# tenstack/batch-scheduler

Hardware: AMD Instinct MI355X
Metric: pod x node fit evals/sec (higher is better)
Workload: dtype int64; 1 GPU; cfg3/tail: 10000 pods / 2000 groups / 5000 nodes, 5 int64 lanes (cpu, mem, eph, pods, gpu), seed 20260921; stages=prefilter+filter+tally+ready, parallelism=single GPU

## Files before the change

### batch-scheduler_amd/build.py

```python
from __future__ import annotations

import os
import shutil
import subprocess

HERE = os.path.dirname(os.path.abspath(__file__))
CSRC = os.path.join(HERE, "csrc")
LIB_DIR = os.environ.get("BS_LIB_DIR") or HERE
PREBUILT_ONLY = bool(os.environ.get("BS_LIB_DIR"))
LIB_PATH = os.path.join(LIB_DIR, "libbsched.so")
_COMMON = ["bs_common.hpp", "bs_kernels.hpp", "bs_nodew_layout.hpp", "bs_lanes.hpp", os.path.join("..", "..", "include", "bsched.h")]
_CTX = _COMMON + ["bs_ctx.hpp", "bs_carve.hpp", "bs_hostmem.hpp", "bs_pod_ranges.hpp"]
_FAST = ["bs_launch.hpp", "bs_fast.hpp", "bs_filter_t.hpp"]
_SEQ = _CTX + ["bs_seq.hpp"]
UNITS = {
    "bsched.hip": _CTX + _FAST + ["bs_epoch.hpp", "bs_queue.hpp", "bs_fdeny.hpp", "bs_sort.hpp", "bs_fit.hpp"],
    "tu_fast.hip": _COMMON + _FAST,
    "tu_seq.hip": _SEQ,
    "tu_seq_expire.hip": _SEQ + ["bs_seq_expire.hpp", "bs_seq_expire_list.hpp"],
    "tu_preempt.hip": _CTX + ["bs_preempt.hpp", "bs_preempt_commit.hpp", "bs_preempt_commit_gang.hpp", "bs_preempt_gang_runs.hpp", "bs_preempt_geom.hpp", "bs_bound_apply.hpp",
                              "bs_bound_nodes.hpp", "bs_bound_nodes_replay.hpp", "bs_pdb.hpp"],
}
SOURCES = list(UNITS)
LATER_UNITS = {
    "tu_wait.hip": _SEQ + ["bs_wait.hpp", "bs_wait_list.hpp", "bs_bound_nodes_replay.hpp"],
}
ALL_UNITS = {**UNITS, **LATER_UNITS}
ALL_SOURCES = list(ALL_UNITS)
LIST_UNITS = {
    "tu_groups.hip": _CTX + ["bs_groups_list.hpp", "bs_groups_list_check.hpp"],
}
BUILD_UNITS = {**ALL_UNITS, **LIST_UNITS}
BUILD_SOURCES = list(BUILD_UNITS)
HEADERS = sorted({h for hs in BUILD_UNITS.values() for h in hs})
OBJ_DIR = os.path.join(HERE, "build")
FLAGS = ["--offload-arch=gfx950", "-O3", "-std=c++17", "-fPIC", "-ffp-contract=off",
         "-fno-fast-math", "-Wall", "-Wno-unused-function"]


def hipcc() -> str:
    exe = shutil.which("hipcc") or "/opt/rocm/bin/hipcc"
    if not os.path.exists(exe):
        raise RuntimeError("hipcc not found: the gfx950 library cannot be built")
    return exe
# ... 103 lines not shown
```

### batch-scheduler_amd/csrc/bs_ctx.hpp

```cpp
#pragma once
#include <rccl/rccl.h>

#include <algorithm>
#include <string>
#include <vector>

#include "bs_carve.hpp"
#include "bs_hostmem.hpp"
#include "bs_kernels.hpp"
#include "bs_lanes.hpp"
#include "bs_pod_ranges.hpp"

namespace bs {

struct EventPair { hipEvent_t a, b; uint32_t id; };

inline size_t align256(size_t x) { return (x + 255) & ~(size_t)255; }
template <class T>
T* at(T* p, size_t n) { return p ? p + n : nullptr; }

struct PodLayout {
  Piece<int32_t> group;
  Piece<int64_t> req;
  Piece<uint32_t> pres, cls, pclass, ppair;
// ... 95 lines not shown
  Piece<uint32_t> off_gmm, off_gsc, off_gmatched, off_gcls, off_gmrpres;
  Piece<uint8_t> off_gflags;
  Piece<int64_t> off_gminres;
  Piece<uint64_t> off_gocc;
  size_t gpack_bytes = 0;
  int32_t info_tag = 0, kinfo_tag = 0;
  bool info_pending = false, kinfo_pending = false;
  uint32_t max_group_cls = 0, max_pod_cls = 0;
  uint32_t h_K = 0;
  uint32_t k_bound = 0;

  uint32_t P = 0;
  DevBuf d_pack[2], d_outpack;
  PodLayout lay[2], stage_lay;
  uint32_t cur_pack = 0;
  bool last_use_classes = false;
  uint32_t map_p = 0;
  DevBuf d_gstat2, d_cdir, d_pdir, d_ckeys, d_cpres, d_pkeys;
  uint32_t gstat_cur = 0;
  uint32_t pair_cap = 0, dir_slots = 0;
  uint32_t ids_used = 0;
  bool rep_valid = false;
  bool dirs_ready = false;
  uint32_t id_room = 0;
  uint32_t serial_insert_max = 2048;
  uint64_t n_applies = 0, n_rederives = 0;
  Piece<uint8_t> off_pf_code, off_fl_code, off_ready;
  Piece<uint32_t> off_pf_first_k, off_fl_feasible, off_fl_slot, off_admit;
  Piece<int32_t> off_pf_leader;
  size_t outpack_bytes = 0;

  DevBuf d_first_elig, d_first_owner, d_first_reject, d_first_pod, d_cap_epoch;
  DevBuf d_epoch, d_nepochs, d_leader_epoch, d_panic_epoch;
  DevBuf d_tcode, d_stage, d_leader_raw, d_first_row, d_first_row64, d_scan_rec, d_feas_rec, d_chunk_rec, d_qreq_s, d_qflags_s, d_qpos;
  DevBuf d_needed, d_qcount, d_ticket, d_desc;
  bool scratch_armed = false;
  bool side_ready = false;
  DevBuf d_tables, d_kp, d_stats, d_fparams, d_fflags, d_chunk_tot, d_blk_scratch, d_gmax, d_chunk_kp;
  DevBuf d_cls_slots, d_cls_rep, d_cls_id, d_qtab_s, d_fu_slot, d_uparams, d_uflags, d_uclaim, d_fu_bitmap, d_fu_feas;
  DevBuf d_nodew;
  bool batch_void = false;
  uint32_t tp_tmin = 768;
  bool no_nodew = false;
  uint32_t slot_keep = 0xFFFFFFFFu;
  uint32_t cls_cap = 0, hash_keep = 0x7FFFFFFFu, n_nominres = 0, scan_slots_cap = 0, filter_slots_cap = 0;
  DevBuf d_fl_bitmap, d_admit, d_ready, d_gcount, d_admit64, d_own_start;
  bool owner_ready = false;
  DevBuf d_order_rank, d_sort;
  uint32_t order_g = 0;
  DevBuf d_gstat, d_pair_next, d_pair_firstq, d_first_reach, d_qstamp_s, d_fast_reject, d_epoch_group;
  bool pairs_ready = false;
  bool bitmap_valid = false;
  bool last_fast = false;
  bool batch_since_pods = false;
  size_t off_hfeas = 0, off_htag = 0;
  uint32_t hstride = 0;
  int32_t host_tag = 0;
  bool last_host_out = false;
  uint32_t no_fast = 0;
  DevBuf d_run_of_epoch, d_run_leader, d_gslot, d_gfirstq;
  bool epochs_ready = false, einfo_pending = false;
  int32_t einfo_tag = 0;
  uint32_t h_R = 0, h_eflags = 0, no_epoch = 0;
  uint32_t last_chain = 0;
  uint32_t last_rows = 0;
  DevBuf d_sq;
// ... 122 lines not shown
```

### batch-scheduler_amd/csrc/bs_fast.hpp

```cpp
#pragma once

#include "bs_kernels.hpp"
#include "bs_filter_t.hpp"

#ifdef BS_NT_TABLES
#define BS_TBL_STORE(p, v) __builtin_nontemporal_store((v), (p))
#else
#define BS_TBL_STORE(p, v) (*(p) = (v))
#endif
namespace bs {

template <bool INL = false>
__device__ __forceinline__ void arm_tally(const GroupsDev& gr, const BatchDev& b, const BatchParams& prm, uint32_t i, uint32_t nthreads);

__device__ __forceinline__ const uint8_t* range_glocal(const BatchDev& b) { return reinterpret_cast<const uint8_t*>(b.pod_ranges); }
__device__ __forceinline__ const uint32_t* range_start(const BatchDev& b, uint32_t G) { return b.pod_ranges + (G + 3u) / 4u; }
__device__ __forceinline__ const uint32_t* range_lfirst(const BatchDev& b, uint32_t G, uint32_t pod_blocks) { return range_start(b, G) + pod_blocks + 1u; }
__device__ __forceinline__ bool range_local_on(const BatchDev& b, const BatchParams& prm) {
  return b.pod_ranges && prm.do_tally && prm.do_ready && !prm.filter_deny;
}

#if BS_EMIT_MAIN
__global__ void k_pods_prep(unsigned long long* tables, uint32_t ntab, uint32_t* gstat, uint32_t ngstat, uint32_t* kcount, uint32_t* gcount, uint32_t G) {
  const uint32_t t = blockIdx.x * blockDim.x + threadIdx.x, nt = gridDim.x * blockDim.x;
// ... 31 lines not shown
  bool winner;
  const uint32_t r = dedupe_insert(slots, mask, hash_keep, h, i, [&](uint32_t o) { return o < pods.p && pods.group[o] == gi && id[rep[o]] == c; }, winner);
  ppair[i] = r;
  if (winner) {
    unsigned long long* head = reinterpret_cast<unsigned long long*>(gstat + (((size_t)3 * G + 1) & ~(size_t)1)) + gi;
    pair_next[i] = atomicExch(head, ((unsigned long long)c << 32) | i);
  }
}
#endif

#if BS_EMIT_MAIN
__global__ void k_groups_apply(const GroupDelta* d, uint32_t n, uint32_t* matched, uint32_t* status_scheduled, uint8_t* flags) {
  const uint32_t t = blockIdx.x * blockDim.x + threadIdx.x;
  if (t >= n) return;
  const GroupDelta x = d[t];
  matched[x.index] = x.matched;
  status_scheduled[x.index] = x.status_scheduled;
  flags[x.index] = (uint8_t)x.flags;
}
#endif

__device__ __forceinline__ void leader_publish(const GroupsDev& gr, const BatchDev& b, uint32_t C, int32_t tag, int32_t* info, int32_t l, int32_t pn,
                                               uint32_t l_matched, uint8_t l_flags, uint32_t l_cls) {
  int32_t steady = -1;
  if (!pn && l >= 0 && C && l_matched > 0 && (l_flags & BS_GROUP_HAS_POD) && l_cls < C) {
    steady = (int32_t)(C + l_cls);
    TableDesc d;
    d.cls = l_cls;
    d.pct = 0.7f;
    b.desc[steady] = d;
  }
  b.leader_epoch[0] = l;
  b.panic_epoch[0] = pn ? 1 : 0;
  __hip_atomic_store(&info[0], l, __ATOMIC_RELAXED, __HIP_MEMORY_SCOPE_SYSTEM);
  __hip_atomic_store(&info[1], pn, __ATOMIC_RELAXED, __HIP_MEMORY_SCOPE_SYSTEM);
  __hip_atomic_store(&info[2], steady, __ATOMIC_RELAXED, __HIP_MEMORY_SCOPE_SYSTEM);
  asm volatile("s_waitcnt vmcnt(0)" ::: "memory");
  __hip_atomic_store(&info[3], tag, __ATOMIC_RELAXED, __HIP_MEMORY_SCOPE_SYSTEM);
}

__device__ __forceinline__ void leader_info_block(const GroupsDev& gr, const BatchDev& b, uint32_t C, int32_t tag, int32_t* info, const DeltaPack& dp,
                                                  uint32_t* matched, uint32_t* status_scheduled, uint8_t* flags) {
  __shared__ unsigned long long s_w[kLeaderBlock / 64];
  __shared__ uint32_t s_slow;
  if (threadIdx.x < dp.n) {
    const GroupDelta x = dp.d[threadIdx.x];
    matched[x.index] = x.matched;
    status_scheduled[x.index] = x.status_scheduled;
    flags[x.index] = (uint8_t)x.flags;
  }
  if (threadIdx.x == 0) s_slow = 0;
  __syncthreads();
  if (!gr.g) {
    if (threadIdx.x == 0) leader_publish(gr, b, C, tag, info, -1, 0, 0u, 0, 0u);
    return;
  }
  if (gr.g <= (uint32_t)kLeaderBlock * kLeaderPerThread) {
    uint32_t f_[kLeaderPerThread], mm_[kLeaderPerThread], sc_[kLeaderPerThread], ma_[kLeaderPerThread], cl_[kLeaderPerThread];
#pragma unroll
    for (int it = 0; it < kLeaderPerThread; ++it) {
      const uint32_t g = threadIdx.x + (uint32_t)it * kLeaderBlock;
      f_[it] = mm_[it] = sc_[it] = ma_[it] = cl_[it] = 0;
      if (g < gr.g) { f_[it] = gr.flags[g]; mm_[it] = gr.min_member[g]; sc_[it] = gr.status_scheduled[g]; ma_[it] = gr.matched[g]; cl_[it] = gr.cls[g]; }
    }
    unsigned long long best = 0;
    bool panic = false;
// ... 125 lines not shown

struct LeaderPre { Res mr; bool have_mr; int64_t min_member, status_scheduled, matched; };
template <bool PUB, typename T>
__device__ __forceinline__ void st_pub(T* p, T v) {
  if constexpr (PUB) __hip_atomic_store(p, v, __ATOMIC_RELAXED, __HIP_MEMORY_SCOPE_AGENT);
  else *p = v;
}
#ifndef BS_HOME_WT
#define BS_HOME_WT 0
#endif
template <typename T>
__device__ __forceinline__ void st_home(T* p, T v) {
#if BS_HOME_WT
  __hip_atomic_store(p, v, __ATOMIC_RELAXED, __HIP_MEMORY_SCOPE_SYSTEM);
#else
  *p = v;
#endif
}
__device__ __forceinline__ uint32_t ld_agent(const uint32_t* p) { return __hip_atomic_load(p, __ATOMIC_RELAXED, __HIP_MEMORY_SCOPE_AGENT); }
__device__ __forceinline__ unsigned long long ld_agent64(const void* p) {
  return __hip_atomic_load(reinterpret_cast<const unsigned long long*>(p), __ATOMIC_RELAXED, __HIP_MEMORY_SCOPE_AGENT);
}
template <int TS>
__device__ __forceinline__ void leader_pre_load(const GroupsDev& gr, int32_t leader, Shape<TS> sh, LeaderPre& o) {
  const uint32_t l = leader >= 0 ? (uint32_t)leader : 0u;
#pragma unroll
  for (uint32_t j = 0; j < BS_MAX_LANES; ++j) o.mr.v[j] = j < sh.L() ? gr.minres[(size_t)j * gr.g + l] : 0;
  o.mr.present = gr.mrpres[l];
  o.have_mr = (gr.flags[l] & BS_GROUP_HAS_MINRES) != 0;
  o.min_member = (int64_t)gr.min_member[l];
  o.status_scheduled = (int64_t)gr.status_scheduled[l];
  o.matched = (int64_t)gr.matched[l];
}
template <int TS>
__device__ __forceinline__ void pre_allocated_from(const LeaderPre& lp, Shape<TS> sh, uint32_t gate, Res& out) {
  res_zero(out, sh);
  const int64_t mm = lp.min_member;
  const int64_t not_finished = lp.matched != 0 ? mm - lp.matched : mm - lp.status_scheduled;
  if (not_finished > 0 && lp.have_mr) {
    Res times;
#pragma unroll
    for (uint32_t j = 0; j < BS_MAX_LANES; ++j)
      if (j < sh.L()) times.v[j] = wmul(lp.mr.v[j], not_finished);
    times.present = lp.mr.present;
    res_add(out, times, sh, gate);
  }
  if (out.v[BS_LANE_PODS] == 0) out.v[BS_LANE_PODS] = mm + 1;
}
template <int TS>
__device__ __forceinline__ uint32_t filter_slot_values(const Res& cur_in, const LeaderPre& lp, Shape<TS> sh, uint32_t gate, int64_t (&R)[4], int64_t (&M)[4]) {
  Res ms, cur = cur_in;
  res_zero(ms, sh);
  res_add(ms, lp.mr, sh, gate);
  res_add(cur, ms, sh, gate);
  uint32_t ff = 0;
#pragma unroll
  for (uint32_t s = 0; s < BS_MAX_SCALARS; ++s) {
    if (s < sh.S()) {
      if ((cur.present & (1u << s)) && cur.v[4 + s] != 0) ff |= 1u;
      if ((ms.present & (1u << s)) && ms.v[4 + s] != 0) ff |= 2u;
    }
  }
#pragma unroll
  for (int j = 0; j < 4; ++j) { R[j] = cur.v[j]; M[j] = ms.v[j]; }
  return ff;
}
// ... 269 lines not shown
                                                 const int64_t* ckeys, const uint32_t* cpres, uint32_t kcap, bool direct = false, uint32_t forced_cls = 0) {
  __shared__ unsigned long long s_wtot[BS_MAX_LANES][4];
  __shared__ uint32_t s_kp[BS_MAX_SCALARS];
  __shared__ unsigned long long s_off[BS_MAX_LANES];
  __shared__ uint32_t s_kpg[BS_MAX_SCALARS];
  __shared__ int64_t s_req[kStepSlotsMax][BS_MAX_LANES];
  __shared__ uint32_t s_qf[kStepSlotsMax];
  __shared__ uint32_t s_first[kStepSlotsMax];
  BS_STAMP(2, 0);
  const Shape<TS> sh(prm.S);
  const uint32_t L = sh.L(), S = sh.S(), LP = prm.LP;
  const uint32_t k = chunk * kTblChunk + threadIdx.x;
  const bool in_range = REGS ? k < nd.n : k < nd.m;
  const uint32_t n = REGS ? (in_range ? k : 0u) : (in_range ? nd.kmap[k] : 0u);
  const TableDesc d = REGS ? TableDesc{forced_cls, 0.7f} : *forced;
  const uint32_t fw = nd.fit[(size_t)d.cls * nd.fit_words + (n >> 5)];
  const uint8_t fl = nd.flags[n];
  const bool valid = in_range && (!REGS || !(fl & BS_NODE_SKIP_MASK));
  const uint32_t ap = nd.apres[n], rp = nd.rpres[n];
  int64_t al[BS_MAX_LANES], rq[BS_MAX_LANES];
#pragma unroll
  for (uint32_t j = 0; j < BS_MAX_LANES; ++j) {
    if (j < L) {
      al[j] = nd.alloc[(size_t)j * nd.stride + n];
      rq[j] = nd.req[(size_t)j * nd.stride + n];
    }
  }
  const uint32_t K = prm.k_host ? prm.k_host : *b.kclass;
  const uint32_t per = (K + nshares - 1u) / nshares, s_lo = share * per, s_hi = min(K, s_lo + per);
  Res raw;
  int32_t leader0 = -1;
  uint8_t panic0 = 0;
  LeaderPre lp0{};
  if constexpr (REGS) {
    const uint32_t cc = s_lo + threadIdx.x < s_hi ? s_lo + threadIdx.x : 0u;
#pragma unroll
    for (uint32_t j = 0; j < BS_MAX_LANES; ++j)
      if (j < L) raw.v[j] = ckeys[(size_t)j * kcap + cc];
    raw.present = cpres[cc];
    leader0 = b.leader_epoch[0];
    panic0 = b.panic_epoch[0];
    if (gr.g) leader_pre_load(gr, leader0, sh, lp0);
  }
  const bool fit = valid && ((fw >> (n & 31u)) & 1u) && !(fl & BS_NODE_TAINT_ERR);
  const uint32_t pres = fit ? (ap & rp) : 0u;
  if (threadIdx.x < BS_MAX_SCALARS) s_kp[threadIdx.x] = BS_INF;
  for (uint32_t t = threadIdx.x; t < kStepSlotsMax; t += kTblChunk) s_first[t] = BS_INF;
  unsigned long long incl[BS_MAX_LANES];
  const int w = wave_id();
#pragma unroll
  for (uint32_t j = 0; j < BS_MAX_LANES; ++j) {
    incl[j] = 0;
    if (j < L) {
      const bool live = fit && (j < 4 || (pres & (1u << (j - 4)))) && !(j == BS_LANE_EPH && !prm.eph_gate);
      const unsigned long long left = live ? (unsigned long long)wsub(scale_f32(al[j], d.pct), rq[j]) : 0ull;
      incl[j] = wave_incl_scan_add_u64(left);
      if (lane_id() == 63) s_wtot[j][w] = incl[j];
    }
  }
  __syncthreads();
#pragma unroll
  for (uint32_t s2 = 0; s2 < BS_MAX_SCALARS; ++s2) {
    if (s2 < S) {
      const unsigned long long mk = __ballot(valid && (pres & (1u << s2)));
      if (mk && lane_id() == 0) atomicMin(&s_kp[s2], chunk * kTblChunk + (uint32_t)(threadIdx.x & ~63u) + (uint32_t)(__ffsll((long long)mk) - 1));
    }
  }
#pragma unroll
  for (uint32_t j = 0; j < BS_MAX_LANES; ++j) {
    if (j < L) {
      unsigned long long off = 0, tot = 0;
#pragma unroll
      for (int i = 0; i < 4; ++i) {
        const unsigned long long x = s_wtot[j][i];
        if (i < w) off += x;
        tot += x;
      }
      incl[j] += off;
      if (threadIdx.x == 0 && share == 0) {
        if constexpr (REGS) {
          const unsigned long long tag = (unsigned long long)prm.seq_inv << 32;
          st_pub<true>(&b.chunk_rec[(size_t)chunk * kRecStride + 2u * j], tag | (uint32_t)tot);
          st_pub<true>(&b.chunk_rec[(size_t)chunk * kRecStride + 2u * j + 1u], tag | (uint32_t)(tot >> 32));
        } else {
          st_pub<true>(&b.chunk_tot[(size_t)chunk * 16 + j], tot);
        }
      }
    }
  }
  __syncthreads();
  __shared__ uint32_t s_ok;
  if constexpr (REGS) {
    if (share == 0 && threadIdx.x < S) st_pub<true>(&b.chunk_rec[(size_t)chunk * kRecStride + 16u + threadIdx.x], ((unsigned long long)prm.seq_inv << 32) | s_kp[threadIdx.x]);
    BS_STAMP(2, 1);
  } else {
    if (share == 0 && threadIdx.x < 16) st_pub<true>(&b.chunk_kp[(size_t)chunk * 16 + threadIdx.x], threadIdx.x < BS_MAX_SCALARS ? s_kp[threadIdx.x] : BS_INF);
    asm volatile("s_waitcnt vmcnt(0)" ::: "memory");
    __syncthreads();
    BS_STAMP(2, 1);
    if (threadIdx.x == 0 && share == 0) (void)__hip_atomic_fetch_add(&b.ticket[kTkTab], 1u, __ATOMIC_RELAXED, __HIP_MEMORY_SCOPE_AGENT);
  }
  if constexpr (REGS) {
    const uint32_t t = s_lo + threadIdx.x;
    if (t < s_hi) {
      uint32_t qf = 0x80000000u;
      Res q;
      res_zero(q, sh);
      if (leader0 >= 0 && !panic0) {
        Res cur;
        res_zero(cur, sh);
        res_add(cur, raw, sh, prm.eph_gate);
        qf = class_scan_query(cur, lp0, sh, prm.eph_gate, q);
      }
      s_qf[threadIdx.x] = qf;
#pragma unroll
      for (uint32_t j = 0; j < BS_MAX_LANES; ++j)
        if (j < L) s_req[threadIdx.x][j] = q.v[j];
    }
  }
  if constexpr (!REGS) {
    if (threadIdx.x == 0) s_ok = (step_wait(&b.ticket[kTkTab], tk_tab0, nchunks, b.h_err) && step_wait(&b.ticket[kTkSlots], tk_pods0, pod_blocks, b.h_err)) ? 1u : 0u;
    __syncthreads();
    BS_STAMP(2, 2);
    if (!s_ok) return;
  }
  {
    const uint32_t ch = (uint32_t)lane_id();
    unsigned long long cv[BS_MAX_LANES];
    uint32_t ckp[BS_MAX_SCALARS];
    if constexpr (REGS) {
      if (w == 0) {
        const uint32_t tagw = prm.seq_inv;
        const unsigned long long* rec = b.chunk_rec + (size_t)(ch < nchunks ? ch : 0u) * kRecStride;
        bool ok = false;
        for (uint32_t spins = 0;; ++spins) {
// ... 128 lines not shown
    BS_STAMP(2, 7);
    return;
  }
  for (uint32_t t = threadIdx.x; t < nmine; t += kTblChunk) {
    if (s_first[t] == BS_INF) continue;
    atomicMin(&b.first_row[s_lo + t], s_first[t]);
  }
  BS_STAMP(2, 7);
}

__device__ __forceinline__ void step_filter_split(uint32_t K, uint32_t W, uint32_t target_waves, uint32_t& tiles, uint32_t& bpw, uint32_t& nchunk) {
  tiles = (2u * K + 63u) / 64u;
  uint32_t nsplit = max(1u, target_waves / max(tiles, 1u));
  nsplit = min(nsplit, max((W + 1u) / 2u, 1u));
  bpw = max(2u, (((W + nsplit - 1u) / nsplit + 1u) / 2u) * 2u);
  nchunk = (W + bpw - 1u) / bpw;
  if ((nchunk + 3u) / 4u > kFeasRecGroups) {
    bpw = ((W + 4u * kFeasRecGroups - 1u) / (4u * kFeasRecGroups) + 1u) / 2u * 2u;
    nchunk = (W + bpw - 1u) / bpw;
  }
}
template <int TS>
__device__ __forceinline__ void step_filter_block(const GroupsDev& gr, const NodesDev& nd, const BatchDev& b, const BatchParams& prm, const int64_t* ckeys,
                                                  const uint32_t* cpres, uint32_t kcap, uint32_t target_waves, uint32_t ustride, uint32_t bx, uint32_t nblocks,
                                                  bool direct, uint32_t tk_slots0, uint32_t slot_producers) {
  __shared__ uint32_t s_cnt[4][64];
  BS_STAMP_AT(4, 0, bx);
  const Shape<TS> sh(prm.S);
  const uint32_t gate = prm.eph_gate, K = prm.k_host ? prm.k_host : (uint32_t)__builtin_amdgcn_readfirstlane((int)*b.kclass), U = 2u * K;
  const uint32_t W = (nd.n + 63u) / 64u;
  if (!U || !W) return;
  uint32_t tiles, bpw, nchunk;
  step_filter_split(K, W, target_waves, tiles, bpw, nchunk);
  const uint32_t groups = (nchunk + 3u) / 4u;
  const int32_t leader0 = b.leader_epoch[0];
  LeaderPre lp0{}, lp1{};
  const bool two = prm.sop_leader0 >= 0 && prm.sop_leader0 != leader0;
  if (gr.g) {
    leader_pre_load(gr, leader0, sh, lp0);
    if (two) leader_pre_load(gr, prm.sop_leader0, sh, lp1); else lp1 = lp0;
  }
  bool waited = false;
  for (uint32_t bi = bx; bi < tiles * groups; bi += nblocks) {
    const uint32_t tile = bi % tiles, group = bi / tiles, chunk = group * 4u + (uint32_t)wave_id();
    const uint32_t src = tile * 64u + (uint32_t)lane_id();
    const bool second = src >= K;
    const uint32_t c = src < U ? (second ? src - K : src) : 0u;
    uint32_t cnt = 0;
    if (chunk < nchunk) {
      Res raw;
#pragma unroll
      for (uint32_t j = 0; j < BS_MAX_LANES; ++j)
        if (j < sh.L()) raw.v[j] = ckeys[(size_t)j * kcap + c];
      raw.present = cpres[c];
      Res cur;
      res_zero(cur, sh);
      res_add(cur, raw, sh, gate);
      LeaderPre lp = lp0;
      if (second) lp = lp1;
      const bool on = src < U && (second ? prm.sop_leader0 >= 0 : leader0 >= 0) && lp.have_mr;
      int64_t R[4], M[4];
      const uint32_t ff = filter_slot_values(cur, lp, sh, gate, R, M);
      filter_item<2, 4, true, true>(nd, b, U, ustride, tile, chunk * bpw, min(W, chunk * bpw + bpw), 0u,
                                    on ? (ff | ((uint32_t)BS_FL_EVALUATED << 8)) : ((uint32_t)BS_FL_NOT_RUN << 8), R, M, &cnt);
    }
    s_cnt[wave_id()][lane_id()] = cnt;
    BS_STAMP_AT(4, 1, bx);
    if (direct && b.h_rows) asm volatile("s_waitcnt vmcnt(0)" ::: "memory");
    __syncthreads();
    BS_STAMP_AT(4, 2, bx);
    if (wave_id() == 0 && src < U) {
      const uint32_t sum = s_cnt[0][lane_id()] + s_cnt[1][lane_id()] + s_cnt[2][lane_id()] + s_cnt[3][lane_id()];
      if (direct) {
        st_pub<true>(&b.feas_rec[(size_t)group * (2u * kStepSlotsMax) + src], ((unsigned long long)prm.seq_inv << 32) | sum);
      } else {
        if (!waited) { (void)step_wait(&b.ticket[kTkSlots], tk_slots0, slot_producers, b.h_err); waited = true; }
        if (sum) atomicAdd(&b.fu_feas[src], sum);
      }
    }
    __syncthreads();
  }
  BS_STAMP_AT(4, 7, bx);
}

template <int TS>
__device__ __forceinline__ void class_slots_block(const GroupsDev& gr, const BatchDev& b, const BatchParams& prm, const int64_t* ckeys, const uint32_t* cpres,
                                                  uint32_t kcap, uint32_t blk, bool zero_feas) {
  const Shape<TS> sh(prm.S);
#ifdef BS_TEST_OLD_ZERO
  zero_feas = true;
#endif
  const uint32_t gate = prm.eph_gate, K = prm.k_host ? prm.k_host : *b.kclass;
  const uint32_t c = blk * kTblChunk + threadIdx.x;
  Res raw;
  const uint32_t cc = c < K ? c : 0u;
#pragma unroll
  for (uint32_t j = 0; j < BS_MAX_LANES; ++j)
    if (j < sh.L()) raw.v[j] = ckeys[(size_t)j * kcap + cc];
  raw.present = cpres[cc];
  const int32_t leader0 = b.leader_epoch[0];
  const uint8_t panic0 = b.panic_epoch[0];
  LeaderPre lp0{}, lp1{};
  const bool two = prm.run_filter && prm.sop_leader0 >= 0 && prm.sop_leader0 != leader0;
  if (gr.g) {
    leader_pre_load(gr, leader0, sh, lp0);
    if (two) leader_pre_load(gr, prm.sop_leader0, sh, lp1); else lp1 = lp0;
  }
  if (c < K) {
    Res cur;
    res_zero(cur, sh);
    res_add(cur, raw, sh, gate);
    if (leader0 >= 0 && !panic0) {
      Res q;
      const uint32_t qfw = class_scan_query(cur, lp0, sh, gate, q);
      int64_t* dst = b.qreq_s + (size_t)c * prm.LP;
#pragma unroll
      for (uint32_t j = 0; j < BS_MAX_LANES; ++j)
        if (j < prm.LP) st_pub<true>(&dst[j], j < sh.L() ? q.v[j] : (int64_t)INT64_MIN);
      st_pub<true>(&b.qflags_s[c], qfw);
      st_pub<true>(&b.qtab_s[c], (int32_t)0);
      st_pub<true>(&b.first_row[c], BS_INF);
      st_pub<true>(&b.qstamp_s[c], prm.stamp);
    }
    if (prm.run_filter) {
      if (leader0 >= 0) filter_slot_from<TS, true>(b, prm, cur, lp0, sh, gate, c, zero_feas);
      if (prm.sop_leader0 >= 0) filter_slot_from<TS, true>(b, prm, cur, lp1, sh, gate, c + K, zero_feas);
    }
  }
  BS_STAMP(1, 4);
  asm volatile("s_waitcnt vmcnt(0)" ::: "memory");
  __syncthreads();
  BS_STAMP(1, 5);
  if (threadIdx.x == 0) (void)__hip_atomic_fetch_add(&b.ticket[kTkSlots], 1u, __ATOMIC_RELAXED, __HIP_MEMORY_SCOPE_AGENT);
}


template <bool INL>
__device__ __forceinline__ void arm_tally(const GroupsDev& gr, const BatchDev& b, const BatchParams& prm, uint32_t i, uint32_t nthreads) {
  if (i == 0) __hip_atomic_store(&b.ticket[1], 0u, __ATOMIC_RELAXED, __HIP_MEMORY_SCOPE_AGENT);
// ... 572 lines not shown
```

### batch-scheduler_amd/csrc/bs_kernels.hpp

```cpp
#pragma once

#include "bs_common.hpp"
#include "bs_nodew_layout.hpp"

namespace bs {

struct NodesDev {
  uint32_t n, stride;
  const int64_t* alloc;
  const int64_t* req;
  const uint32_t* apres;
  const uint32_t* rpres;
  const uint8_t* flags;
  const uint32_t* fit;
  uint32_t fit_words, n_classes;
  const uint32_t* kmap;
  uint32_t m;
  const int64_t* left4;
  const int64_t* lglob;
};

struct GroupsDev {
  uint32_t g;
  const uint32_t* min_member;
  const uint32_t* status_scheduled;
  const uint32_t* matched;
  const uint8_t* flags;
  const uint32_t* cls;
  const int64_t* minres;
  const uint32_t* mrpres;
  const uint64_t* occupied;
};

struct PodsDev {
  uint32_t p;
// ... 13 lines not shown
inline uint32_t cdiv(uint32_t a, uint32_t b) { return (a + b - 1) / b; }

struct BoundLayout { size_t boff, prio, start, group, id, req, pres, pdb, nviol; };
__host__ __device__ inline size_t bound_layout(uint32_t L, uint32_t N, uint32_t B, BoundLayout& b) {
  const size_t nB = B ? B : 1u, nN = N ? N : 1u, m = ~(size_t)255;
  size_t o = 0;
  b.boff = o; o = (o + ((size_t)N + 1) * 4 + 255) & m;
  b.prio = o; o = (o + nB * 4 + 255) & m;
  b.start = o; o = (o + nB * 8 + 255) & m;
  b.group = o; o = (o + nB * 4 + 255) & m;
  b.id = o; o = (o + nB * 4 + 255) & m;
  b.req = o; o = (o + nB * L * 8 + 255) & m;
  b.pres = o; o = (o + nB * 4 + 255) & m;
  b.pdb = o; o = (o + nB + 255) & m;
  b.nviol = o; o = (o + nN * 4 + 255) & m;
  return o;
}

constexpr uint8_t ST_ELIG = 1;
constexpr uint8_t ST_REACH6 = 2;
constexpr uint8_t ST_OWNED = 4;
constexpr uint8_t ST_QUERY = 8;

struct BatchDev {
  uint32_t* first_elig;
  uint32_t* first_owner;
  uint32_t* first_reject;
  uint32_t* first_pod;
  uint32_t* cap_epoch;
  uint32_t* epoch;
  uint32_t* nepochs;
  int32_t* leader_epoch;
  uint8_t* panic_epoch;
  uint8_t* tcode;
  uint8_t* stage;
  int32_t* leader_raw;
  uint32_t* first_row;
  unsigned long long* chunk_rec;
  unsigned long long* first_row64;
  unsigned long long* scan_rec;
  unsigned long long* feas_rec;
  int64_t* qreq_s;
  uint32_t* qflags_s;
  uint32_t* qpos;
  uint32_t* needed;
  uint32_t* qcount;
  uint32_t* ticket;
  TableDesc* desc;
  uint32_t* ntables;
  int64_t* tables;
  uint32_t* kp;
  uint64_t* stats;
  unsigned long long* chunk_tot;
  uint32_t* chunk_kp;
  uint32_t* blk_scratch;
  int64_t* gmax;
  int64_t* fparams;
  uint32_t* fflags;
  const uint32_t* pclass;
  const uint32_t* kclass;
  unsigned long long* cls_slots;
  uint32_t cls_mask;
  int32_t* qtab_s;
  uint32_t* fu_slot;
  int64_t* uparams;
  uint32_t* uflags;
// ... 1467 lines not shown
BS_DEF_FILTER_POD2(1, 1, 0, 0, 0)
BS_DEF_FILTER_POD2(2, 0, 1, 0, 0)
BS_DEF_FILTER_POD2(3, 1, 1, 0, 0)
BS_DEF_FILTER_POD2(4, 0, 0, 1, 0)
BS_DEF_FILTER_POD2(5, 1, 0, 1, 0)
BS_DEF_FILTER_POD2(6, 0, 1, 1, 0)
BS_DEF_FILTER_POD2(7, 1, 1, 1, 0)
BS_DEF_FILTER_POD2(8, 0, 0, 0, 1)
BS_DEF_FILTER_POD2(9, 1, 0, 0, 1)
BS_DEF_FILTER_POD2(10, 0, 1, 0, 1)
BS_DEF_FILTER_POD2(11, 1, 1, 0, 1)
BS_DEF_FILTER_POD2(12, 0, 0, 1, 1)
BS_DEF_FILTER_POD2(13, 1, 0, 1, 1)
BS_DEF_FILTER_POD2(14, 0, 1, 1, 1)
BS_DEF_FILTER_POD2(15, 1, 1, 1, 1)

template <int MASK, int PU = 4>
__device__ __forceinline__ void filter_pod_loop(uint32_t np, const int64_t (*sR)[4], const unsigned long long (&okmask)[2],
                                                const int64_t (&l)[2][4], uint32_t (&vlo)[2], uint32_t (&vhi)[2]) {
  for (uint32_t pp = 0; pp < np; pp += PU) {
    int64_t R[PU][4];
#pragma unroll
    for (int u = 0; u < PU; ++u) {
      const uint32_t pu = min(pp + (uint32_t)u, np - 1);
#pragma unroll
      for (int j = 0; j < 4; ++j) R[u][j] = ((MASK >> j) & 1) ? sR[pu][j] : 0;
    }
#pragma unroll
    for (int u = 0; u < PU; ++u)
      filter_pod2<MASK>(min(pp + (uint32_t)u, np - 1), R[u], okmask[0], okmask[1], l[0], l[1], vlo[0], vhi[0], vlo[1], vhi[1]);
  }
}

template <int NB, int PU = 4, bool DB = true, bool REGS = false>
__device__ __forceinline__ void filter_item(const NodesDev& nd, const BatchDev& b, uint32_t U, uint32_t ustride, uint32_t ptile,
                                            uint32_t w0, uint32_t w1, uint32_t stamp = 0, uint32_t ff_in = 0, const int64_t* R_in = nullptr,
                                            const int64_t* M_in = nullptr, uint32_t* cnt_out = nullptr) {
  static_assert(NB == 2, "the inner statement handles two node blocks");
  typedef const __attribute__((address_space(4))) uint32_t* cflag_t;
  const int lane = lane_id();
  const uint32_t p0 = ptile * 64u;
  const uint32_t np = min(64u, U - p0);

  const bool mine = (uint32_t)lane < np;
  const uint32_t src = p0 + (uint32_t)lane;
  uint32_t myff = (uint32_t)BS_FL_NOT_RUN << 8;
  int64_t M[4] = {0, 0, 0, 0}, myR[4] = {0, 0, 0, 0};
  if constexpr (REGS) {
    if (mine) {
      myff = ff_in;
#pragma unroll
      for (int j = 0; j < 4; ++j) { myR[j] = R_in[j]; M[j] = M_in[j]; }
    }
  } else if (mine) {
    myff = b.uflags[src];
    const int64_t* rs = b.uparams + (size_t)src * 8;
#pragma unroll
    for (int j = 0; j < 4; ++j) { myR[j] = rs[j]; M[j] = rs[4 + j]; }
  }
  int64_t gl[8];
#pragma unroll
  for (int j = 0; j < 8; ++j) gl[j] = nd.lglob[j];
  int64_t l[NB][4], ln[NB][4];
  uint8_t nfl[NB], nfln[NB];
  auto load_blocks = [&](uint32_t w, int64_t (&dst)[NB][4], uint8_t (&fl)[NB]) {
#pragma unroll
    for (int nb = 0; nb < NB; ++nb) {
      const uint32_t n = (w + nb) * 64u + (uint32_t)lane;
      const bool nvalid = (w + nb) < w1 && n < nd.n;
      fl[nb] = 0xFF;
#pragma unroll
      for (int j = 0; j < 4; ++j) dst[nb][j] = INT64_MIN;
      if (nvalid) {
#pragma unroll
        for (int j = 0; j < 4; ++j) dst[nb][j] = nd.left4[(size_t)j * nd.stride + n];
        fl[nb] = nd.flags[n];
      }
    }
  };
  load_blocks(w0, l, nfl);
  if (!REGS && stamp) myff = (myff >> 16) == stamp ? (myff & 0xFFFFu) : ((uint32_t)BS_FL_NOT_RUN << 8);
  const uint32_t myfl = myff >> 8;
  const bool ev = myfl == BS_FL_EVALUATED;
  if (!ev) {
#pragma unroll
    for (int j = 0; j < 4; ++j) M[j] = 0;
  }
  __shared__ int64_t s_R[4][64][4];
  __builtin_amdgcn_wave_barrier();
  uint32_t lane_mask = 0;
  bool tile_allfail = false;
  {
#pragma unroll
    for (int j = 0; j < 4; ++j) s_R[wave_id()][lane][j] = myR[j];
    __builtin_amdgcn_wave_barrier();
    const bool c2pod = ev && !(myff & 1u);
    const unsigned long long c2mask = __ballot(c2pod);
#pragma unroll
    for (int j = 0; j < 4; ++j) {
      if (__ballot(c2pod && !(gl[j] >= myR[j]))) lane_mask |= 1u << j;
      if (c2mask && !__ballot(c2pod && gl[4 + j] >= myR[j])) tile_allfail = true;
    }
  }
  const unsigned long long evmask = __ballot(ev);
  if (!evmask) return;
  bool uniformM = true;
  int64_t M0[4] = {0, 0, 0, 0};
  uint32_t lb0 = 0;
  if (evmask) {
    const int first = __ffsll((long long)evmask) - 1;
    bool same = true;
#pragma unroll
    for (int j = 0; j < 4; ++j) {
// ... 331 lines not shown
```

### batch-scheduler_amd/csrc/bsched.hip

```cpp
#include <dlfcn.h>
#include <hip/hip_runtime.h>

#include <algorithm>
#include <cstdio>
#include <cstdlib>
#include <cstring>
#include <new>
#include <string>
#include <vector>

#ifndef BS_UNITY
#define BS_TU_MAIN
#endif
#include "bs_ctx.hpp"
#include "bs_fast.hpp"
#include "bs_epoch.hpp"
#include "bs_sort.hpp"
#include "bs_fit.hpp"
#include "bs_queue.hpp"
#include "bs_fdeny.hpp"
#include "bs_launch.hpp"
#ifdef BS_UNITY
#include "tu_fast.hip"
#include "tu_seq.hip"
// ... 57 lines not shown
    if (_rc) return _rc;                                       \
    __VA_ARGS__;                                               \
    LAUNCHCHK(ctx, id);                                        \
    _rc = timer_end(ctx, _slot, st);                           \
    if (_rc) return _rc;                                       \
  } while (0)
#define TIMED(ctx, id, ...) TIMED_ON(ctx, id, (hipStream_t) nullptr, __VA_ARGS__)

void advance_batch_seq(bs_ctx* c) {
  c->batch_seq++;
  c->stamp_ctr = (c->stamp_ctr + 1u) % 65535u;
  if (c->key_seq >= 0xFFFFFFFEu) { c->key_seq = 1; c->rekey_pending = true; }
  else c->key_seq++;
}

int flush_groups(bs_ctx* c);
template <class D>
void pod_cols(D& p, const PodLayout& l, void* pk) {
  p.group = l.group.in(pk); p.req = l.req.in(pk); p.pres = l.pres.in(pk); p.cls = l.cls.in(pk); p.owner = l.owner.in(pk); p.flags = l.flags.in(pk);
}
uint32_t* ppair_dev(const bs_ctx* c) { return c->lay[c->cur_pack].ppair.in(c->d_pack[c->cur_pack].p); }
uint32_t* gstat_dev(const bs_ctx* c) { return (c->gstat_cur ? c->d_gstat2 : c->d_gstat).as<uint32_t>(); }
BatchDev batch_dev(const bs_ctx* c) {
  BatchDev b{};
  b.first_elig = c->d_first_elig.as<uint32_t>();
  b.first_owner = c->d_first_owner.as<uint32_t>();
  b.first_reject = c->d_first_reject.as<uint32_t>();
  b.first_pod = c->d_first_pod.as<uint32_t>();
  b.cap_epoch = c->d_cap_epoch.as<uint32_t>();
  b.epoch = c->d_epoch.as<uint32_t>();
  b.nepochs = c->d_nepochs.as<uint32_t>();
  b.leader_epoch = c->d_leader_epoch.as<int32_t>();
  b.panic_epoch = c->d_panic_epoch.as<uint8_t>();
  b.tcode = c->d_tcode.as<uint8_t>();
  b.stage = c->d_stage.as<uint8_t>();
  b.leader_raw = c->d_leader_raw.as<int32_t>();
  b.first_row = c->d_first_row.as<uint32_t>();
  b.first_row64 = c->d_first_row64.as<unsigned long long>();
  b.scan_rec = c->d_scan_rec.as<unsigned long long>();
  b.feas_rec = c->d_feas_rec.as<unsigned long long>();
  b.chunk_rec = c->d_chunk_rec.as<unsigned long long>();
  b.qreq_s = c->d_qreq_s.as<int64_t>();
  b.qflags_s = c->d_qflags_s.as<uint32_t>();
  b.qpos = c->d_qpos.as<uint32_t>();
  b.needed = c->d_needed.as<uint32_t>();
  b.qcount = c->d_qcount.as<uint32_t>();
  b.ticket = c->d_ticket.as<uint32_t>();
  b.gcount = c->d_gcount.as<uint32_t>();
  b.own_start = c->d_own_start.as<uint32_t>();
  b.admit64 = c->d_admit64.as<unsigned long long>();
  b.desc = c->d_desc.as<TableDesc>();
  b.tables = c->d_tables.as<int64_t>();
  b.kp = c->d_kp.as<uint32_t>();
  b.stats = c->d_stats.as<uint64_t>();
  b.chunk_tot = c->d_chunk_tot.as<unsigned long long>();
  b.blk_scratch = c->d_blk_scratch.as<uint32_t>();
  b.gmax = c->d_gmax.as<int64_t>();
  b.chunk_kp = c->d_chunk_kp.as<uint32_t>();
  b.fparams = c->d_fparams.as<int64_t>();
  b.fflags = c->d_fflags.as<uint32_t>();
  b.pclass = pclass_dev(c);
  b.kclass = at(c->d_nepochs.as<uint32_t>(), 2);
  b.cls_slots = c->d_cls_slots.as<unsigned long long>();
  b.cls_mask = c->cls_cap ? c->cls_cap - 1 : 0;
  b.qtab_s = c->d_qtab_s.as<int32_t>();
  b.uparams = c->d_uparams.as<int64_t>();
// ... 640 lines not shown
int bs_create(const bs_config* cfg, bs_ctx** out) {
  if (!cfg || !out) return BS_ERR_INVALID;
  *out = nullptr;
  if (cfg->abi_version != BS_ABI_VERSION || cfg->scalar_lanes > BS_MAX_SCALARS) return BS_ERR_INVALID;
  int ndev = 0;
  if (hipGetDeviceCount(&ndev) != hipSuccess || ndev <= 0 || cfg->device < 0 || cfg->device >= ndev) return BS_ERR_NO_DEVICE;
  hipDeviceProp_t prop;
  if (hipGetDeviceProperties(&prop, cfg->device) != hipSuccess) return BS_ERR_NO_DEVICE;
  if (std::strncmp(prop.gcnArchName, "gfx950", 6) != 0) return BS_ERR_NO_DEVICE;
  bs_ctx* c = new (std::nothrow) bs_ctx();
  if (!c) return BS_ERR_NOMEM;
  c->cfg = *cfg;
  c->S = cfg->scalar_lanes;
  c->L = BS_FIXED_LANES + c->S;
  c->LP = c->S == 0 ? 4 : (c->S <= 4 ? 8 : 16);
  if (hipSetDevice(cfg->device) != hipSuccess || hipStreamCreateWithFlags(&c->stream.h, hipStreamNonBlocking) != hipSuccess ||
      hipStreamCreateWithFlags(&c->stream3.h, hipStreamNonBlocking) != hipSuccess ||
      hipEventCreateWithFlags(&c->ev_query.h, hipEventDisableTiming) != hipSuccess ||
      hipEventCreateWithFlags(&c->ev_filter.h, hipEventDisableTiming) != hipSuccess) {
    delete c;
    return BS_ERR_NO_DEVICE;
  }
  if (c->d_nepochs.reserve(64) != hipSuccess || hipMemset(c->d_nepochs.p, 0, 64) != hipSuccess || c->d_ticket.reserve(kTkWords * 4) != hipSuccess ||
      hipMemset(c->d_ticket.p, 0, kTkWords * 4) != hipSuccess) {
    delete c;
    return BS_ERR_NOMEM;
  }
  if (c->d_info.reserve(64) != hipSuccess || c->d_first_reach.reserve(64) != hipSuccess || hipMemset(c->d_first_reach.p, 0xFF, 64) != hipSuccess ||
      c->h_info.reserve(64) != hipSuccess) {
    delete c;
    return BS_ERR_NOMEM;
  }
  std::memset(c->h_info.p, 0, 64);
  c->batch_seq = 1;
  read_env_switches(c);
  *out = c;
  return BS_OK;
}

int bs_destroy(bs_ctx* c) {
  if (!c) return BS_OK;
  if (c->host_probe && c->hp_n)
    std::fprintf(stderr, "[bs host probe] %llu fast-chain batches: to chain choice %.2f us | to launch A %.2f | launch A call %.2f | to launch B %.2f | launch B call %.2f | rest %.2f\n",
                 (unsigned long long)c->hp_n, c->hp_ns[0] / 1e3 / c->hp_n, c->hp_ns[1] / 1e3 / c->hp_n, c->hp_ns[2] / 1e3 / c->hp_n, c->hp_ns[3] / 1e3 / c->hp_n,
                 c->hp_ns[4] / 1e3 / c->hp_n, c->hp_ns[5] / 1e3 / c->hp_n);
  (void)hipSetDevice(c->cfg.device);
  (void)hipStreamSynchronize(c->stream);
  (void)hipStreamSynchronize(c->stream3);
  for (auto& e : c->events) { (void)hipEventDestroy(e.a); (void)hipEventDestroy(e.b); }
  if (c->comm && c->rccl_destroy) (void)c->rccl_destroy((ncclComm_t)c->comm);
  delete c;
  return BS_OK;
}

int bs_nodes_load(bs_ctx* c, const bs_nodes_soa* nodes) {
  if (c) c->seq_wait_valid = false;
  if (!c || !nodes) return BS_ERR_INVALID;
  int rc = use_device(c);
  if (rc) return rc;
  if ((rc = settle_pending(c))) return rc;
  c->steady_prev = -1;
  const uint32_t N = nodes->n, L = c->L;
  if (N && (!nodes->allocatable || !nodes->requested || !nodes->allocatable_present || !nodes->requested_present || !nodes->flags))
    return BS_ERR_INVALID;
  if (N > 0x7FFFFFF0u) return BS_ERR_CAPACITY;
  c->N = N;
// ... 2131 lines not shown
```

Baseline: 3736 billion evals/s.

## Publish leader record as one cache line and prefetch next filter item

The kernel that picks the epoch leader now also writes a 128-byte LeaderRec holding the leader's minres, flags and counters. Downstream filter and tally kernels read that record with one coalesced per-lane load plus readlane, instead of doing several scattered group-table loads after the leader is known. The step filter loop also loads the next item's pod keys and node blocks into registers before processing the current one, and it peeks at the slot ticket so it can skip the wait when the producers are already done. The cost is more register pressure and extra code paths, with a fallback to the full load whenever the record does not match the leader or the lane count is too large.

```diff
diff --git a/batch-scheduler_amd/build.py b/batch-scheduler_amd/build.py
--- a/batch-scheduler_amd/build.py
+++ b/batch-scheduler_amd/build.py
@@ -9,7 +9,7 @@
 LIB_DIR = os.environ.get("BS_LIB_DIR") or HERE
 PREBUILT_ONLY = bool(os.environ.get("BS_LIB_DIR"))
 LIB_PATH = os.path.join(LIB_DIR, "libbsched.so")
-_COMMON = ["bs_common.hpp", "bs_kernels.hpp", "bs_nodew_layout.hpp", "bs_lanes.hpp", os.path.join("..", "..", "include", "bsched.h")]
+_COMMON = ["bs_common.hpp", "bs_kernels.hpp", "bs_nodew_layout.hpp", "bs_leader_rec.hpp", "bs_lanes.hpp", os.path.join("..", "..", "include", "bsched.h")]
 _CTX = _COMMON + ["bs_ctx.hpp", "bs_carve.hpp", "bs_hostmem.hpp", "bs_pod_ranges.hpp"]
 _FAST = ["bs_launch.hpp", "bs_fast.hpp", "bs_filter_t.hpp"]
 _SEQ = _CTX + ["bs_seq.hpp"]
diff --git a/batch-scheduler_amd/csrc/bs_ctx.hpp b/batch-scheduler_amd/csrc/bs_ctx.hpp
--- a/batch-scheduler_amd/csrc/bs_ctx.hpp
+++ b/batch-scheduler_amd/csrc/bs_ctx.hpp
@@ -151,6 +151,7 @@
 
   DevBuf d_first_elig, d_first_owner, d_first_reject, d_first_pod, d_cap_epoch;
   DevBuf d_epoch, d_nepochs, d_leader_epoch, d_panic_epoch;
+  DevBuf d_leader_rec;
   DevBuf d_tcode, d_stage, d_leader_raw, d_first_row, d_first_row64, d_scan_rec, d_feas_rec, d_chunk_rec, d_qreq_s, d_qflags_s, d_qpos;
   DevBuf d_needed, d_qcount, d_ticket, d_desc;
   bool scratch_armed = false;
diff --git a/batch-scheduler_amd/csrc/bs_fast.hpp b/batch-scheduler_amd/csrc/bs_fast.hpp
--- a/batch-scheduler_amd/csrc/bs_fast.hpp
+++ b/batch-scheduler_amd/csrc/bs_fast.hpp
@@ -87,6 +87,21 @@
   }
   b.leader_epoch[0] = l;
   b.panic_epoch[0] = pn ? 1 : 0;
+  if (b.leader_rec) {
+    LeaderRec r{};
+    r.leader = l;
+    r.panic = pn ? 1u : 0u;
+    if (l >= 0) {
+#pragma unroll
+      for (uint32_t j = 0; j < kLeaderRecLanes; ++j) r.minres[j] = j < b.leader_rec_lanes ? gr.minres[(size_t)j * gr.g + (uint32_t)l] : 0;
+      r.mrpres = gr.mrpres[l];
+      r.flags = gr.flags[l];
+      r.min_member = gr.min_member[l];
+      r.status_scheduled = gr.status_scheduled[l];
+      r.matched = gr.matched[l];
+    }
+    *b.leader_rec = r;
+  }
   __hip_atomic_store(&info[0], l, __ATOMIC_RELAXED, __HIP_MEMORY_SCOPE_SYSTEM);
   __hip_atomic_store(&info[1], pn, __ATOMIC_RELAXED, __HIP_MEMORY_SCOPE_SYSTEM);
   __hip_atomic_store(&info[2], steady, __ATOMIC_RELAXED, __HIP_MEMORY_SCOPE_SYSTEM);
@@ -278,6 +293,41 @@
   o.status_scheduled = (int64_t)gr.status_scheduled[l];
   o.matched = (int64_t)gr.matched[l];
 }
+__device__ __forceinline__ uint32_t leader_rec_fetch(const BatchDev& b) { return reinterpret_cast<const uint32_t*>(b.leader_rec)[lane_id() & 31]; }
+__device__ __forceinline__ uint32_t lane_word(uint32_t w, int lane) { return (uint32_t)__builtin_amdgcn_readlane((int)w, lane); }
+template <int TS>
+__device__ __forceinline__ void leader_pre_from_words(uint32_t w, Shape<TS> sh, LeaderPre& o) {
+#pragma unroll
+  for (uint32_t j = 0; j < BS_MAX_LANES; ++j) {
+    o.mr.v[j] = 0;
+    if (j < kLeaderRecLanes && j < sh.L())
+      o.mr.v[j] = (int64_t)(((unsigned long long)lane_word(w, kLrMinres + 2 * (int)j + 1) << 32) | lane_word(w, kLrMinres + 2 * (int)j));
+  }
+  o.mr.present = lane_word(w, kLrMrpres);
+  o.have_mr = (lane_word(w, kLrFlags) & BS_GROUP_HAS_MINRES) != 0;
+  o.min_member = (int64_t)lane_word(w, kLrMinMember);
+  o.status_scheduled = (int64_t)lane_word(w, kLrScheduled);
+  o.matched = (int64_t)lane_word(w, kLrMatched);
+}
+template <int TS>
+__device__ __forceinline__ bool leader_pre_from_rec(uint32_t w, int32_t leader0, Shape<TS> sh, LeaderPre& o) {
+  if (sh.L() > kLeaderRecLanes || (int32_t)lane_word(w, kLrLeader) != leader0) return false;
+  leader_pre_from_words(w, sh, o);
+  return true;
+}
+__device__ __forceinline__ uint32_t leader_live_fetch(const GroupsDev& gr, int32_t leader, uint32_t L, uint32_t& flags) {
+  const uint32_t l = leader >= 0 ? (uint32_t)leader : 0u;
+  const int i = lane_id() & 31;
+  const uint32_t j = min((uint32_t)(i >= kLrMinres ? (i - kLrMinres) >> 1 : 0), min(L, kLeaderRecLanes) - 1u);
+  const uint32_t* p = reinterpret_cast<const uint32_t*>(gr.minres + (size_t)j * gr.g + l) + (i >= kLrMinres ? (i - kLrMinres) & 1 : 0);
+  if (i == kLrMrpres) p = gr.mrpres + l;
+  if (i == kLrMinMember) p = gr.min_member + l;
+  if (i == kLrScheduled) p = gr.status_scheduled + l;
+  if (i == kLrMatched) p = gr.matched + l;
+  flags = gr.flags[l];
+  return *p;
+}
+__device__ __forceinline__ uint32_t leader_live_words(uint32_t w, uint32_t flags) { return lane_id() == kLrFlags ? flags : w; }
 template <int TS>
 __device__ __forceinline__ void pre_allocated_from(const LeaderPre& lp, Shape<TS> sh, uint32_t gate, Res& out) {
   res_zero(out, sh);
@@ -613,6 +663,7 @@
   int32_t leader0 = -1;
   uint8_t panic0 = 0;
   LeaderPre lp0{};
+  uint32_t lrec = 0;
   if constexpr (REGS) {
     const uint32_t cc = s_lo + threadIdx.x < s_hi ? s_lo + threadIdx.x : 0u;
 #pragma unroll
@@ -621,7 +672,7 @@
     raw.present = cpres[cc];
     leader0 = b.leader_epoch[0];
     panic0 = b.panic_epoch[0];
-    if (gr.g) leader_pre_load(gr, leader0, sh, lp0);
+    lrec = leader_rec_fetch(b);
   }
   const bool fit = valid && ((fw >> (n & 31u)) & 1u) && !(fl & BS_NODE_TAINT_ERR);
   const uint32_t pres = fit ? (ap & rp) : 0u;
@@ -682,6 +733,7 @@
     if (threadIdx.x == 0 && share == 0) (void)__hip_atomic_fetch_add(&b.ticket[kTkTab], 1u, __ATOMIC_RELAXED, __HIP_MEMORY_SCOPE_AGENT);
   }
   if constexpr (REGS) {
+    if (!leader_pre_from_rec(lrec, leader0, sh, lp0) && gr.g) leader_pre_load(gr, leader0, sh, lp0);
     const uint32_t t = s_lo + threadIdx.x;
     if (t < s_hi) {
       uint32_t qf = 0x80000000u;
@@ -876,27 +928,44 @@
   if (!U || !W) return;
   uint32_t tiles, bpw, nchunk;
   step_filter_split(K, W, target_waves, tiles, bpw, nchunk);
-  const uint32_t groups = (nchunk + 3u) / 4u;
+  const uint32_t groups = (nchunk + 3u) / 4u, items = tiles * groups;
+  auto item_fetch = [&](uint32_t bi, Res& raw, FilterPre<2>& pre) {
+    const uint32_t tile = bi % tiles, chunk = min((bi / tiles) * 4u + (uint32_t)wave_id(), nchunk - 1u);
+    const uint32_t src = tile * 64u + (uint32_t)lane_id();
+    const uint32_t c = src < U ? (src >= K ? src - K : src) : 0u;
+#pragma unroll
+    for (uint32_t j = 0; j < BS_MAX_LANES; ++j)
+      if (j < sh.L()) raw.v[j] = ckeys[(size_t)j * kcap + c];
+    raw.present = cpres[c];
+    filter_item_preload<2>(nd, chunk * bpw, min(W, chunk * bpw + bpw), pre);
+  };
+  if (bx >= items) return;
   const int32_t leader0 = b.leader_epoch[0];
+  const uint32_t lrec = leader_rec_fetch(b);
+  const bool carried = prm.sop_leader0 >= 0 && gr.g;
+  uint32_t lfl = 0;
+  const uint32_t llive = carried ? leader_live_fetch(gr, prm.sop_leader0, sh.L(), lfl) : 0u;
+  Res raw0;
+  FilterPre<2> pre0;
+  item_fetch(bx, raw0, pre0);
   LeaderPre lp0{}, lp1{};
-  const bool two = prm.sop_leader0 >= 0 && prm.sop_leader0 != leader0;
-  if (gr.g) {
-    leader_pre_load(gr, leader0, sh, lp0);
-    if (two) leader_pre_load(gr, prm.sop_leader0, sh, lp1); else lp1 = lp0;
+  const bool two = carried && prm.sop_leader0 != leader0;
+  if (!leader_pre_from_rec(lrec, leader0, sh, lp0) && gr.g) leader_pre_load(gr, leader0, sh, lp0);
+  if (two) {
+    if (sh.L() <= kLeaderRecLanes) leader_pre_from_words(leader_live_words(llive, lfl), sh, lp1);
+    else leader_pre_load(gr, prm.sop_leader0, sh, lp1);
+  } else {
+    lp1 = lp0;
   }
   bool waited = false;
-  for (uint32_t bi = bx; bi < tiles * groups; bi += nblocks) {
+  auto item = [&](uint32_t bi, const Res& raw, const FilterPre<2>& pre) {
     const uint32_t tile = bi % tiles, group = bi / tiles, chunk = group * 4u + (uint32_t)wave_id();
     const uint32_t src = tile * 64u + (uint32_t)lane_id();
     const bool second = src >= K;
-    const uint32_t c = src < U ? (second ? src - K : src) : 0u;
     uint32_t cnt = 0;
+    uint32_t tk_look = tk_slots0;
+    if (!direct && !waited && wave_id() == 0) tk_look = ld_agent(&b.ticket[kTkSlots]);
     if (chunk < nchunk) {
-      Res raw;
-#pragma unroll
-      for (uint32_t j = 0; j < BS_MAX_LANES; ++j)
-        if (j < sh.L()) raw.v[j] = ckeys[(size_t)j * kcap + c];
-      raw.present = cpres[c];
       Res cur;
       res_zero(cur, sh);
       res_add(cur, raw, sh, gate);
@@ -906,7 +975,7 @@
       int64_t R[4], M[4];
       const uint32_t ff = filter_slot_values(cur, lp, sh, gate, R, M);
       filter_item<2, 4, true, true>(nd, b, U, ustride, tile, chunk * bpw, min(W, chunk * bpw + bpw), 0u,
-                                    on ? (ff | ((uint32_t)BS_FL_EVALUATED << 8)) : ((uint32_t)BS_FL_NOT_RUN << 8), R, M, &cnt);
+                                    on ? (ff | ((uint32_t)BS_FL_EVALUATED << 8)) : ((uint32_t)BS_FL_NOT_RUN << 8), R, M, &cnt, &pre);
     }
     s_cnt[wave_id()][lane_id()] = cnt;
     BS_STAMP_AT(4, 1, bx);
@@ -918,11 +987,20 @@
       if (direct) {
         st_pub<true>(&b.feas_rec[(size_t)group * (2u * kStepSlotsMax) + src], ((unsigned long long)prm.seq_inv << 32) | sum);
       } else {
-        if (!waited) { (void)step_wait(&b.ticket[kTkSlots], tk_slots0, slot_producers, b.h_err); waited = true; }
+        if (!waited) {
+          if ((uint32_t)(tk_look - tk_slots0) < slot_producers) (void)step_wait(&b.ticket[kTkSlots], tk_slots0, slot_producers, b.h_err);
+          waited = true;
+        }
         if (sum) atomicAdd(&b.fu_feas[src], sum);
       }
     }
     __syncthreads();
+  };
+  Res raw = raw0;
+  FilterPre<2> pre = pre0;
+  for (uint32_t bi = bx; bi < items; bi += nblocks) {
+    item(bi, raw, pre);
+    if (bi + nblocks < items) item_fetch(bi + nblocks, raw, pre);
   }
   BS_STAMP_AT(4, 7, bx);
 }
@@ -944,11 +1022,18 @@
   raw.present = cpres[cc];
   const int32_t leader0 = b.leader_epoch[0];
   const uint8_t panic0 = b.panic_epoch[0];
+  const uint32_t lrec = leader_rec_fetch(b);
+  const bool carried = prm.run_filter && prm.sop_leader0 >= 0 && gr.g;
+  uint32_t lfl = 0;
+  const uint32_t llive = carried ? leader_live_fetch(gr, prm.sop_leader0, sh.L(), lfl) : 0u;
   LeaderPre lp0{}, lp1{};
-  const bool two = prm.run_filter && prm.sop_leader0 >= 0 && prm.sop_leader0 != leader0;
-  if (gr.g) {
-    leader_pre_load(gr, leader0, sh, lp0);
-    if (two) leader_pre_load(gr, prm.sop_leader0, sh, lp1); else lp1 = lp0;
+  const bool two = carried && prm.sop_leader0 != leader0;
+  if (!leader_pre_from_rec(lrec, leader0, sh, lp0) && gr.g) leader_pre_load(gr, leader0, sh, lp0);
+  if (two) {
+    if (sh.L() <= kLeaderRecLanes) leader_pre_from_words(leader_live_words(llive, lfl), sh, lp1);
+    else leader_pre_load(gr, prm.sop_leader0, sh, lp1);
+  } else {
+    lp1 = lp0;
   }
   if (c < K) {
     Res cur;
diff --git a/batch-scheduler_amd/csrc/bs_kernels.hpp b/batch-scheduler_amd/csrc/bs_kernels.hpp
--- a/batch-scheduler_amd/csrc/bs_kernels.hpp
+++ b/batch-scheduler_amd/csrc/bs_kernels.hpp
@@ -1,6 +1,7 @@
 #pragma once
 
 #include "bs_common.hpp"
+#include "bs_leader_rec.hpp"
 #include "bs_nodew_layout.hpp"
 
 namespace bs {
@@ -80,6 +81,8 @@
   uint32_t* nepochs;
   int32_t* leader_epoch;
   uint8_t* panic_epoch;
+  LeaderRec* leader_rec;
+  uint32_t leader_rec_lanes;
   uint8_t* tcode;
   uint8_t* stage;
   int32_t* leader_raw;
@@ -1613,10 +1616,35 @@
   }
 }
 
+template <int NB>
+struct FilterPre { int64_t gl[8]; int64_t l[NB][4]; uint8_t nfl[NB]; };
+template <int NB>
+__device__ __forceinline__ void filter_load_blocks(const NodesDev& nd, uint32_t w, uint32_t w1, int64_t (&dst)[NB][4], uint8_t (&fl)[NB]) {
+  const int lane = lane_id();
+#pragma unroll
+  for (int nb = 0; nb < NB; ++nb) {
+    const uint32_t n = (w + nb) * 64u + (uint32_t)lane;
+    const bool nvalid = (w + nb) < w1 && n < nd.n;
+    fl[nb] = 0xFF;
+#pragma unroll
+    for (int j = 0; j < 4; ++j) dst[nb][j] = INT64_MIN;
+    if (nvalid) {
+#pragma unroll
+      for (int j = 0; j < 4; ++j) dst[nb][j] = nd.left4[(size_t)j * nd.stride + n];
+      fl[nb] = nd.flags[n];
+    }
+  }
+}
+template <int NB>
+__device__ __forceinline__ void filter_item_preload(const NodesDev& nd, uint32_t w0, uint32_t w1, FilterPre<NB>& o) {
+#pragma unroll
+  for (int j = 0; j < 8; ++j) o.gl[j] = nd.lglob[j];
+  filter_load_blocks<NB>(nd, w0, w1, o.l, o.nfl);
+}
 template <int NB, int PU = 4, bool DB = true, bool REGS = false>
 __device__ __forceinline__ void filter_item(const NodesDev& nd, const BatchDev& b, uint32_t U, uint32_t ustride, uint32_t ptile,
                                             uint32_t w0, uint32_t w1, uint32_t stamp = 0, uint32_t ff_in = 0, const int64_t* R_in = nullptr,
-                                            const int64_t* M_in = nullptr, uint32_t* cnt_out = nullptr) {
+                                            const int64_t* M_in = nullptr, uint32_t* cnt_out = nullptr, const FilterPre<NB>* pre = nullptr) {
   static_assert(NB == 2, "the inner statement handles two node blocks");
   typedef const __attribute__((address_space(4))) uint32_t* cflag_t;
   const int lane = lane_id();
@@ -1641,7 +1669,7 @@
   }
   int64_t gl[8];
 #pragma unroll
-  for (int j = 0; j < 8; ++j) gl[j] = nd.lglob[j];
+  for (int j = 0; j < 8; ++j) gl[j] = REGS ? pre->gl[j] : nd.lglob[j];
   int64_t l[NB][4], ln[NB][4];
   uint8_t nfl[NB], nfln[NB];
   auto load_blocks = [&](uint32_t w, int64_t (&dst)[NB][4], uint8_t (&fl)[NB]) {
@@ -1659,7 +1687,16 @@
       }
     }
   };
-  load_blocks(w0, l, nfl);
+  if constexpr (REGS) {
+#pragma unroll
+    for (int nb = 0; nb < NB; ++nb) {
+      nfl[nb] = pre->nfl[nb];
+#pragma unroll
+      for (int j = 0; j < 4; ++j) l[nb][j] = pre->l[nb][j];
+    }
+  } else {
+    load_blocks(w0, l, nfl);
+  }
   if (!REGS && stamp) myff = (myff >> 16) == stamp ? (myff & 0xFFFFu) : ((uint32_t)BS_FL_NOT_RUN << 8);
   const uint32_t myfl = myff >> 8;
   const bool ev = myfl == BS_FL_EVALUATED;
diff --git a/batch-scheduler_amd/csrc/bs_leader_rec.hpp b/batch-scheduler_amd/csrc/bs_leader_rec.hpp
--- /dev/null
+++ b/batch-scheduler_amd/csrc/bs_leader_rec.hpp
@@ -0,0 +1,26 @@
+#pragma once
+#include <cstddef>
+#include <cstdint>
+
+#include "../../include/bsched.h"
+
+namespace bs {
+
+constexpr uint32_t kLeaderRecLanes = BS_FIXED_LANES + 4;
+constexpr int kLeaderRecFill = 0x80;
+
+struct alignas(128) LeaderRec {
+  int32_t leader;
+  uint32_t panic;
+  int64_t minres[kLeaderRecLanes];
+  uint32_t mrpres, flags, min_member, status_scheduled, matched;
+  uint32_t pad[9];
+};
+static_assert(sizeof(LeaderRec) == 128 && alignof(LeaderRec) == 128, "one cache line");
+static_assert(offsetof(LeaderRec, leader) == 0 && offsetof(LeaderRec, panic) == 4 && offsetof(LeaderRec, minres) == 8, "the readers take the record word by word");
+static_assert(offsetof(LeaderRec, mrpres) == 72 && offsetof(LeaderRec, flags) == 76 && offsetof(LeaderRec, min_member) == 80, "the readers take the record word by word");
+static_assert(offsetof(LeaderRec, status_scheduled) == 84 && offsetof(LeaderRec, matched) == 88, "the readers take the record word by word");
+constexpr int kLrLeader = 0, kLrPanic = 1, kLrMinres = 2, kLrMrpres = 18, kLrFlags = 19, kLrMinMember = 20, kLrScheduled = 21, kLrMatched = 22;
+static_assert(kLrMinres + 2 * (int)kLeaderRecLanes == kLrMrpres && kLrMatched < 32, "word indices follow the struct");
+
+}
diff --git a/batch-scheduler_amd/csrc/bsched.hip b/batch-scheduler_amd/csrc/bsched.hip
--- a/batch-scheduler_amd/csrc/bsched.hip
+++ b/batch-scheduler_amd/csrc/bsched.hip
@@ -113,6 +113,8 @@
   b.nepochs = c->d_nepochs.as<uint32_t>();
   b.leader_epoch = c->d_leader_epoch.as<int32_t>();
   b.panic_epoch = c->d_panic_epoch.as<uint8_t>();
+  b.leader_rec = c->d_leader_rec.as<LeaderRec>();
+  b.leader_rec_lanes = std::min<uint32_t>(c->L, kLeaderRecLanes);
   b.tcode = c->d_tcode.as<uint8_t>();
   b.stage = c->d_stage.as<uint8_t>();
   b.leader_raw = c->d_leader_raw.as<int32_t>();
@@ -819,6 +821,10 @@
     return BS_ERR_NOMEM;
   }
   std::memset(c->h_info.p, 0, 64);
+  if (reserve_filled(c, c->d_leader_rec, sizeof(LeaderRec), kLeaderRecFill) != BS_OK) {
+    delete c;
+    return BS_ERR_NOMEM;
+  }
   c->batch_seq = 1;
   read_env_switches(c);
   *out = c;
```

Result: slower. 3673 billion evals/s (-1.7%).
